# li-kunyi/CUT3R-SLAM

Measured on AMD Instinct MI355X. Metric: frames/sec (ViT pointmap + covisibility-graph tracking step) on 640x480, higher is better.
Workload: dtype f16

## Files before the change

### cut3r_slam_amd/csrc/attention.hip

```cpp
#include <atomic>
#include <cmath>
#include <cstdlib>
#include <type_traits>
#include "common.h"
#include "../../include/cut3r_hip.h"

namespace {

typedef __fp16 fp16x4_t __attribute__((ext_vector_type(4)));

DEVINL void halves(float x, float& lo, float& hi) {
    const auto r = __builtin_amdgcn_permlane32_swap(__float_as_uint(x), __float_as_uint(x), false, false);
    lo = __uint_as_float(r[0]);
    hi = __uint_as_float(r[1]);
}

struct AttnArgs {
    const h16* q; const h16* k; const h16* v; h16* o;
    int Nq, Nk;
    long long q_sb, q_sn, k_sb, k_sn, v_sb, v_sn, o_sb, o_sn;
    float scale_log2;
};

template <int D, int NW>
__global__ __launch_bounds__(NW * 64, (D <= 64 && NW == 4) ? 3 : 1) void attn_kernel(const AttnArgs a) {
    constexpr int NTHR = NW * 64;
    constexpr int KT = 64;
    constexpr int DQ = D / 16;
    constexpr int DP = (D + 31) / 32;
    constexpr int KS_LD = D + 8;
    constexpr int VS_BYTES = (64 * DP) % 128 == 0 ? 64 * DP + 64 : 64 * DP;
    constexpr int V_LD = VS_BYTES / 2;
    constexpr int CHUNKS = KT * (D / 8);
    constexpr int NCH = (CHUNKS + NTHR - 1) / NTHR;
    __shared__ __attribute__((aligned(16))) h16 Ks[KT * KS_LD];
    __shared__ __attribute__((aligned(16))) h16 Vs[KT * V_LD];

    const int tid = threadIdx.x, lane = tid & 63, wave = tid >> 6;
    const int r = lane & 31, hh = lane >> 5;
    const int h = blockIdx.y, b = blockIdx.z;
    const int q0 = blockIdx.x * (32 * NW) + wave * 32;
    const h16* qp = a.q + (size_t)b * a.q_sb + (size_t)h * D;
    const h16* kp = a.k + (size_t)b * a.k_sb + (size_t)h * D;
    const h16* vp = a.v + (size_t)b * a.v_sb + (size_t)h * D;

    for (int i = tid; i < KT * V_LD; i += NTHR) Vs[i] = (h16)0;

    half8_t qf[DQ];
    {
        int qr = q0 + r;
        if (qr > a.Nq - 1) qr = a.Nq - 1;
        const h16* qrow = qp + (size_t)qr * a.q_sn;
#pragma unroll
        for (int s = 0; s < DQ; s++) qf[s] = *reinterpret_cast<const half8_t*>(qrow + 16 * s + 8 * hh);
    }

    f32x16 ot[DP];
#pragma unroll
    for (int d = 0; d < DP; d++)
#pragma unroll
        for (int i = 0; i < 16; i++) ot[d][i] = 0.f;
    float m_run = -INFINITY, l_run = 0.f;
    const bool active = q0 < a.Nq;
    const int extra = (a.Nk > KT && (a.Nk % KT) == 1) ? 1 : 0;
    if (extra) {
        float dot = 0.f;
#pragma unroll
        for (int s = 0; s < DQ; s++) {
            const half8_t k0 = *reinterpret_cast<const half8_t*>(kp + 16 * s + 8 * hh);
#pragma unroll
            for (int j = 0; j < 8; j++) dot = fmaf((float)qf[s][j], (float)k0[j], dot);
        }
        { float d0, d1; halves(dot, d0, d1); dot = d0 + d1; }
        m_run = dot * a.scale_log2;
        l_run = hh == 0 ? 1.f : 0.f;
#pragma unroll
        for (int d = 0; d < DP; d++)
#pragma unroll
            for (int g4 = 0; g4 < 4; g4++) {
                const int dd = d * 32 + 8 * g4 + 4 * hh;
                if (dd < D) {
                    const half4_t v0 = *reinterpret_cast<const half4_t*>(vp + dd);
#pragma unroll
                    for (int e = 0; e < 4; e++) ot[d][4 * g4 + e] = (float)v0[e];
                }
            }
    }

    half8_t rk[NCH], rv[NCH];
    const h16* kptr[NCH];
    const h16* vptr[NCH];
    int kkey[NCH];
#pragma unroll
    for (int c = 0; c < NCH; c++) {
        const int id = tid + c * NTHR;
        const int key = id / (D / 8), ch = id - key * (D / 8);
        kkey[c] = key;
        kptr[c] = kp + (size_t)(extra + key) * a.k_sn + ch * 8;
        vptr[c] = vp + (size_t)(extra + key) * a.v_sn + ch * 8;
    }
    auto load_kv = [&](int t) {
        const int kbase = extra + t * KT;
        const bool full = kbase + KT <= a.Nk;
#pragma unroll
        for (int c = 0; c < NCH; c++) {
// ... 35 lines not shown
        half8_t kf[2][DQ];
#pragma unroll
        for (int kt2 = 0; kt2 < 2; kt2++)
#pragma unroll
            for (int s = 0; s < DQ; s++) kf[kt2][s] = *reinterpret_cast<const half8_t*>(&Ks[(kt2 * 32 + r) * KS_LD + 16 * s + 8 * hh]);
        __builtin_amdgcn_sched_barrier(0);
#pragma unroll
        for (int kt2 = 0; kt2 < 2; kt2++) {
#pragma unroll
            for (int i = 0; i < 16; i++) st[kt2][i] = 0.f;
#pragma unroll
            for (int s = 0; s < DQ; s++) st[kt2] = __builtin_amdgcn_mfma_f32_32x32x16_f16(kf[kt2][s], qf[s], st[kt2], 0, 0, 0);
        }
        const int kbase = extra + t * KT;
        float mloc = -INFINITY;
        if (kbase + KT <= a.Nk) {
#pragma unroll
            for (int kt2 = 0; kt2 < 2; kt2++)
#pragma unroll
                for (int i = 0; i < 16; i++) mloc = fmaxf(mloc, st[kt2][i]);
        } else {
#pragma unroll
            for (int kt2 = 0; kt2 < 2; kt2++)
#pragma unroll
                for (int i = 0; i < 16; i++) {
                    const int key = kbase + kt2 * 32 + (i & 3) + 8 * (i >> 2) + 4 * hh;
                    const float sv = key < a.Nk ? st[kt2][i] : -INFINITY;
                    st[kt2][i] = sv;
                    mloc = fmaxf(mloc, sv);
                }
        }
        { float m0_, m1_; halves(mloc, m0_, m1_); mloc = fmaxf(m0_, m1_) * a.scale_log2; }
        const float m_new = fmaxf(m_run, mloc);
        const bool grew = m_new > m_run;
        const float alpha = __builtin_amdgcn_exp2f(m_run - m_new);
        m_run = m_new;
        float lsum = 0.f;
#pragma unroll
        for (int kt2 = 0; kt2 < 2; kt2++)
#pragma unroll
            for (int i = 0; i < 16; i++) {
                const float p = __builtin_amdgcn_exp2f(fmaf(st[kt2][i], a.scale_log2, -m_new));
                st[kt2][i] = p;
                lsum += p;
            }
        l_run = l_run * alpha + lsum;
        if (__any(grew)) {
#pragma unroll
            for (int d = 0; d < DP; d++)
#pragma unroll
                for (int i = 0; i < 16; i++) ot[d][i] *= alpha;
        }

        const int g16 = lane >> 4, j16 = lane & 15;
#pragma unroll
        for (int kt2 = 0; kt2 < 2; kt2++)
#pragma unroll
            for (int s2 = 0; s2 < 2; s2++) {
                half8_t pf;
#pragma unroll
                for (int j = 0; j < 8; j++) pf[j] = (h16)st[kt2][8 * s2 + j];
#pragma unroll
                for (int d = 0; d < DP; d++) {
                    const int k0 = kt2 * 32 + 16 * s2 + 4 * (g16 >> 1);
                    const int c0 = d * 32 + 16 * (g16 & 1);
                    const h16* vp = &Vs[(k0 + (j16 >> 2)) * V_LD + c0 + 4 * (j16 & 3)];
                    const fp16x4_t lo = __builtin_amdgcn_ds_read_tr16_b64_v4f16((__attribute__((address_space(3))) fp16x4_t*)(vp));
                    const fp16x4_t hi = __builtin_amdgcn_ds_read_tr16_b64_v4f16((__attribute__((address_space(3))) fp16x4_t*)(vp + 8 * V_LD));
                    half8_t vf;
                    __builtin_memcpy(&vf, &lo, 8);
                    __builtin_memcpy(reinterpret_cast<char*>(&vf) + 8, &hi, 8);
                    ot[d] = __builtin_amdgcn_mfma_f32_32x32x16_f16(vf, pf, ot[d], 0, 0, 0);
                }
            }
    }

    float l0_, l1_;
    halves(l_run, l0_, l1_);
    const float l_tot = l0_ + l1_;
    const float inv = 1.0f / l_tot;
    const int qr = q0 + r;
    if (qr < a.Nq) {
        h16* orow = a.o + (size_t)b * a.o_sb + (size_t)qr * a.o_sn + (size_t)h * D;
#pragma unroll
        for (int d = 0; d < DP; d++)
#pragma unroll
            for (int g4 = 0; g4 < 4; g4++) {
                int dd = d * 32 + 8 * g4 + 4 * hh;
                if (dd < D) {
                    half4_t o = {(h16)(ot[d][4 * g4 + 0] * inv), (h16)(ot[d][4 * g4 + 1] * inv), (h16)(ot[d][4 * g4 + 2] * inv),
                                 (h16)(ot[d][4 * g4 + 3] * inv)};
                    *reinterpret_cast<half4_t*>(orow + dd) = o;
                }
            }
    }
}


DEVINL void dma_piece(const char* gbase , unsigned voff, unsigned lds ) {
    asm volatile("s_mov_b32 m0, %2\n\ts_nop 0\n\tglobal_load_lds_dwordx4 %0, %1" ::"v"(voff), "s"(gbase), "s"(lds) : "memory", "m0");
}
DEVINL unsigned lds_addr(const void* p) {
    return (unsigned)(unsigned long long)(__attribute__((address_space(3))) const void*)p;
}

template <int N>
DEVINL void wait_vm() { asm volatile("s_waitcnt vmcnt(%0)" ::"n"(N) : "memory"); }
template <int P, int MAXT>
DEVINL void wait_tiles_ahead(int tiles_ahead) {
    if constexpr (MAXT == 0) wait_vm<0>();
    else {
        if (tiles_ahead >= MAXT) wait_vm<P * MAXT>();
        else wait_tiles_ahead<P, MAXT - 1>(tiles_ahead);
    }
}

template <int D, int QB, int NST, int NW>
__global__ __launch_bounds__(64 * NW, (QB == 1 ? 2 : 1)) void attn_pipe_kernel(const AttnArgs a, const int nblk, const int HB, const int H) {
    constexpr int KT = 64;
    constexpr int PPW = 8 / NW;
    constexpr int AHEAD = NST - 4;
    constexpr int DQ = D / 16;
    constexpr int DP = (D + 31) / 32;
    constexpr int CH = D / 8;
    constexpr int VOFF = KT * 128;
    constexpr int STAGE = 2 * KT * 128;
    static_assert(D % 16 == 0 && D <= 64 && NST >= 4 && (NW == 4 || NW == 8), "head dims 16..64; the ring holds tiles j-1 .. j+2 and NST-4 more in flight");
    __shared__ __attribute__((aligned(1024))) unsigned char smem[NST * STAGE];

    const int tid = threadIdx.x, lane = tid & 63;
    const int wave = __builtin_amdgcn_readfirstlane(tid >> 6);
    const int r = lane & 31, hh = lane >> 5;
    const int L = blockIdx.x;
    const int xb = (L >> 3) % nblk;
    const int bh = ((L >> 3) / nblk) * 8 + (L & 7);
    if (bh >= HB) return;
    const int h = bh % H, b = bh / H;
    const int q0 = xb * (32 * NW * QB) + wave * (32 * QB);
    const h16* qp = a.q + (size_t)b * a.q_sb + (size_t)h * D;
    const h16* kp = a.k + (size_t)b * a.k_sb + (size_t)h * D;
    const h16* vp = a.v + (size_t)b * a.v_sb + (size_t)h * D;
    const bool active = q0 < a.Nq;
    const int extra = (a.Nk > KT && (a.Nk % KT) == 1) ? 1 : 0;
    const int ntiles = (a.Nk - extra + KT - 1) / KT;

    if (CH < 8) {
        for (int i = tid; i < NST * STAGE / 16; i += 64 * NW) *reinterpret_cast<f32x4*>(smem + i * 16) = f32x4{0.f, 0.f, 0.f, 0.f};
        asm volatile("s_waitcnt lgkmcnt(0)" ::: "memory");
        asm volatile("s_barrier" ::: "memory");
    }

    auto lane_src = [&](int c, int row_limit, unsigned& ko, unsigned& vo, bool& kval, bool& vval) {
        const int row = (wave * PPW + c) * 8 + (lane >> 3), slot = lane & 7;
        const int kc = slot ^ ((row >> 1) & 7), vc = slot ^ (((row >> 1) & 1) << 2);
        const int rr = min(row, row_limit);
        ko = (unsigned)rr * (unsigned)(a.k_sn * 2) + kc * 16;
        vo = (unsigned)rr * (unsigned)(a.v_sn * 2) + vc * 16;
        kval = kc < CH;
        vval = vc < CH;
    };
    unsigned koffb[PPW], voffb[PPW];
#pragma unroll
    for (int c = 0; c < PPW; c++) {
        bool kv_, vv_;
        lane_src(c, KT - 1, koffb[c], voffb[c], kv_, vv_);
    }
    const char* ktile = reinterpret_cast<const char*>(kp + (size_t)extra * a.k_sn);
    const char* vtile = reinterpret_cast<const char*>(vp + (size_t)extra * a.v_sn);
    int st_issue = 0;
    auto issue = [&](int t) {
        if (t >= ntiles) return;
        unsigned char* st = smem + st_issue * STAGE;
        st_issue = st_issue + 1 == NST ? 0 : st_issue + 1;
        const int left = a.Nk - (extra + t * KT);
#pragma unroll
        for (int c = 0; c < PPW; c++) {
            unsigned ko = koffb[c], vo = voffb[c];
// ... 190 lines not shown
                    __builtin_amdgcn_sched_group_barrier(0x008, 1, 0);
                    __builtin_amdgcn_sched_group_barrier(0x100, 2, 0);
                    __builtin_amdgcn_sched_group_barrier(0x002, 9, 0);
                }
            }
            int gflag = grew ? 1 : 0;
#pragma unroll
            for (int qb = 0; qb < QB; qb++) {
                typedef unsigned u32x4 __attribute__((ext_vector_type(4)));
                u32x4 p0, p1, p2, p3;
                __builtin_memcpy(&p0, &P[PAR][qb][0][0], 16);
                __builtin_memcpy(&p1, &P[PAR][qb][0][1], 16);
                __builtin_memcpy(&p2, &P[PAR][qb][1][0], 16);
                __builtin_memcpy(&p3, &P[PAR][qb][1][1], 16);
                asm volatile("" : "+v"(gflag) : "v"(p0), "v"(p1), "v"(p2), "v"(p3), "v"(l_run[qb]));
            }
            if (__any(gflag)) {
#pragma unroll
                for (int qb = 0; qb < QB; qb++)
#pragma unroll
                    for (int d = 0; d < DP; d++)
#pragma unroll
                        for (int i = 0; i < 16; i++) ot[qb][d][i] *= alpha[qb];
            }
        }
    };
    using T0 = std::integral_constant<int, 0>;
    using T1 = std::integral_constant<int, 1>;
    using Y = std::true_type;
    using N = std::false_type;

#pragma unroll
    for (int t = 0; t < NST - 3; t++) issue(t);
    {
        wait_tiles_ahead<2 * PPW, AHEAD>(ntiles - 1);
        asm volatile("s_barrier" ::: "memory");
        issue(NST - 3);
        {
            half8_t kf[2][DQ];
#pragma unroll
            for (int kt2 = 0; kt2 < 2; kt2++)
#pragma unroll
                for (int s = 0; s < DQ; s++) kf[kt2][s] = *reinterpret_cast<const half8_t*>(smem + kt2 * 32 * 128 + koff[s]);
#pragma unroll
            for (int kt2 = 0; kt2 < 2; kt2++)
#pragma unroll
                for (int qb = 0; qb < QB; qb++) {
#pragma unroll
                    for (int i = 0; i < 16; i++) S[0][qb][kt2][i] = 0.f;
#pragma unroll
                    for (int s = 0; s < DQ; s++) S[0][qb][kt2] = __builtin_amdgcn_mfma_f32_32x32x16_f16(kf[kt2][s], qf[qb][s], S[0][qb][kt2], 0, 0, 0);
                }
        }
    }
    const bool ragged = extra + ntiles * KT > a.Nk;
    if (ntiles > 1) step(T0{}, N{}, Y{}, Y{}, N{}, 0);
    else if (ragged) step(T0{}, N{}, N{}, Y{}, Y{}, 0);
    else step(T0{}, N{}, N{}, Y{}, N{}, 0);
    int j = 1;
    for (; j + 2 < ntiles; j += 2) {
        step(T1{}, Y{}, Y{}, Y{}, N{}, j);
        step(T0{}, Y{}, Y{}, Y{}, N{}, j + 1);
    }
    if (j + 1 < ntiles) { step(T1{}, Y{}, Y{}, Y{}, N{}, j); j++; }
    if (ntiles > 1) {
        if (ragged) {
            if (j & 1) step(T1{}, Y{}, N{}, Y{}, Y{}, j); else step(T0{}, Y{}, N{}, Y{}, Y{}, j);
        } else {
            if (j & 1) step(T1{}, Y{}, N{}, Y{}, N{}, j); else step(T0{}, Y{}, N{}, Y{}, N{}, j);
        }
        j++;
    }
    if (j & 1) step(T1{}, Y{}, N{}, N{}, N{}, j); else step(T0{}, Y{}, N{}, N{}, N{}, j);

#pragma unroll
    for (int qb = 0; qb < QB; qb++) {
        float l0_, l1_;
        halves(l_run[qb], l0_, l1_);
        const float l_tot = l0_ + l1_;
        const float inv = 1.0f / l_tot;
        const int qr = q0 + qb * 32 + r;
        if (qr < a.Nq) {
            h16* orow = a.o + (size_t)b * a.o_sb + (size_t)qr * a.o_sn + (size_t)h * D;
#pragma unroll
            for (int d = 0; d < DP; d++)
#pragma unroll
                for (int g4 = 0; g4 < 4; g4++) {
                    int dd = d * 32 + 8 * g4 + 4 * hh;
                    if (dd < D) {
                        half4_t o = {(h16)(ot[qb][d][4 * g4 + 0] * inv), (h16)(ot[qb][d][4 * g4 + 1] * inv), (h16)(ot[qb][d][4 * g4 + 2] * inv),
                                     (h16)(ot[qb][d][4 * g4 + 3] * inv)};
                        *reinterpret_cast<half4_t*>(orow + dd) = o;
                    }
                }
        }
    }
}

std::atomic<int> g_attn_variant{[] { const char* e = getenv("CUT3R_ATTN_PIPE"); return e ? atoi(e) : 1; }()};

int attn_instance(int B, int H, int Nq, int D) {
    static const long long nw4_min = [] { const char* e = getenv("CUT3R_ATTN_NW4_MIN"); return e ? atoll(e) : 384LL; }();
    if (D != 16 && D != 32 && D != 48 && D != 64 && D != 128) return 0;
    if ((D == 48 || D == 64) && g_attn_variant.load(std::memory_order_relaxed) != 0) return 104;
    const long long blocks128 = (long long)B * H * ((Nq + 127) / 128);
    return (blocks128 >= nw4_min || D >= 128) ? 4 : 2;
}

template <int D>
int launch_attn(const AttnArgs& a, int B, int H, hipStream_t s) {
    const int inst = attn_instance(B, H, a.Nq, D);
    if constexpr (D == 48 || D == 64) {
        if (inst == 104) {
            const int nblk = (a.Nq + 127) / 128, HB = H * B;
            dim3 grid((unsigned)(((HB + 7) / 8) * 8 * nblk));
            hipLaunchKernelGGL((attn_pipe_kernel<D, 1, 4, 4>), grid, dim3(256), 0, s, a, nblk, HB, H);
            return cut3r_check_launch();
        }
    }
    if (inst == 4) {
        dim3 grid((a.Nq + 127) / 128, H, B);
        hipLaunchKernelGGL((attn_kernel<D, 4>), grid, dim3(256), 0, s, a);
    } else if (inst == 2) {
        dim3 grid((a.Nq + 63) / 64, H, B);
        hipLaunchKernelGGL((attn_kernel<D, 2>), grid, dim3(128), 0, s, a);
    } else {
        return CUT3R_ERR_ARG;
    }
    return cut3r_check_launch();
}

}

extern "C" int cut3r_attention_variant(int v) {
    if (v < 0) return g_attn_variant.load(std::memory_order_relaxed);
    return g_attn_variant.exchange(v ? 1 : 0, std::memory_order_relaxed);
}

extern "C" int cut3r_attention_kernel_for(int B, int H, int Nq, int D) {
    if (B <= 0 || H <= 0 || Nq <= 0) return 0;
    return attn_instance(B, H, Nq, D);
}

extern "C" int cut3r_attention_f16(const void* q, const void* k, const void* v, void* out, int B, int H, int Nq, int Nk, int D,
                                   long long q_sb, long long q_sn, long long k_sb, long long k_sn, long long v_sb, long long v_sn,
                                   long long o_sb, long long o_sn, float scale, void* stream) {
    if (!q || !k || !v || !out || B <= 0 || H <= 0 || Nq <= 0 || Nk <= 0) return CUT3R_ERR_ARG;
    if (((uintptr_t)q | (uintptr_t)k | (uintptr_t)v) & 15) return CUT3R_ERR_ARG;
    if ((uintptr_t)out & 7) return CUT3R_ERR_ARG;
    if ((q_sn | k_sn | v_sn | q_sb | k_sb | v_sb) & 7) return CUT3R_ERR_ARG;
    if ((o_sn | o_sb) & 3) return CUT3R_ERR_ARG;
    if (!(scale > 0.f) || !std::isfinite(scale)) return CUT3R_ERR_ARG;
    AttnArgs a;
    a.q = (const h16*)q; a.k = (const h16*)k; a.v = (const h16*)v; a.o = (h16*)out;
    a.Nq = Nq; a.Nk = Nk;
    a.q_sb = q_sb; a.q_sn = q_sn; a.k_sb = k_sb; a.k_sn = k_sn; a.v_sb = v_sb; a.v_sn = v_sn; a.o_sb = o_sb; a.o_sn = o_sn;
    a.scale_log2 = scale * 1.44269504088896340736f;
    hipStream_t s = (hipStream_t)stream;
    switch (D) {
        case 16: return launch_attn<16>(a, B, H, s);
        case 32: return launch_attn<32>(a, B, H, s);
        case 48: return launch_attn<48>(a, B, H, s);
        case 64: return launch_attn<64>(a, B, H, s);
        case 128: return launch_attn<128>(a, B, H, s);
        default: return CUT3R_ERR_ARG;
    }
}
```

### cut3r_slam_amd/csrc/gemm.hip

```cpp
#include <cstdlib>
#include "common.h"
#include "dpt_tail.h"
#include "../../include/cut3r_hip.h"

namespace {

constexpr int BK = 64;
constexpr int KCH = BK / 8;

struct GemmArgs {
    const h16* A; const h16* B; void* C;
    const float* bias; const void* res1; const void* res2;
    int M, N, K, lda, ldb, ldc, ldr1, ldr2;
    int act, out_f16, res1_f16, res2_f16;
    long long sA, sB, sC, sBias, sR1, sR2;
    int conv_k, H, W, Cin, cstride, Ho, Wo, relu_in;
    int shuf, shuf_cout, shuf_Hin, shuf_Win;
    int swz;
    int prio;
    const long long* rope_pos; const float* rope_table; int rope_cols, rope_pmin, rope_npos, rope_d;
    const float* ln_stats; const float* ln_c; int ln_nslab; float ln_eps;
    float* stats_out; h16* out16; int ld16;
    const float* dpt_w; const float* dpt_b; float* dpt_pts; float* dpt_conf; long long dpt_pts_vs, dpt_conf_vs;
};
// ... 522 lines not shown
    }
#pragma unroll
    for (int p = 0; p < EPI_PASSES; p++) {
        f32x4 r1v[PF];
        auto load_r1 = [&](int i) {
            const int r = r0 + i * RPP;
            const int gm = m0 + p * EPI_ROWS + r;
            return (r < EPI_ROWS && gm < M) ? load_res4(g.res1, g.res1_f16, (size_t)z * g.sR1 + (size_t)gm * g.ldr1 + gn) : zero4;
        };
        if (plain && col_ok && g.res1) {
#pragma unroll
            for (int i = 0; i < PF; i++) r1v[i] = load_r1(i);
        }
        if (p > 0) __syncthreads();
#pragma unroll
        for (int i = 0; i < MT; i++)
#pragma unroll
            for (int j = 0; j < NT; j++)
#pragma unroll
                for (int e = 0; e < 4; e++) {
                    const int r = wm * WM + i * 16 + fq * 4 + e - p * EPI_ROWS;
                    const int c = wn * WN + j * 16 + fr;
                    if (EPI_PASSES == 1 || (r >= 0 && r < EPI_ROWS)) cs[r * CPAD + c] = acc[i][j][e];
                }
        __syncthreads();
        if (col_ok) {
            if (plain) {
#pragma unroll
                for (int i = 0; i < ITER; i++) {
                    const int r = r0 + i * RPP;
                    const int gm = m0 + p * EPI_ROWS + r;
                    f32x4 r1 = zero4;
                    if (g.res1) {
                        r1 = r1v[i % PF];
                        if (i + PF < ITER) r1v[i % PF] = load_r1(i + PF);
                    }
                    if (r < EPI_ROWS && gm < M) {
                        const f32x4 r2 = g.res2 ? load_res4(g.res2, g.res2_f16, (size_t)z * g.sR2 + (size_t)gm * g.ldr2 + gn) : zero4;
                        f32x4 v = *reinterpret_cast<const f32x4*>(cs + r * CPAD + c4);
                        if (g.ln_stats) v = ln_pre4(v, lnp[2 * (p * EPI_ROWS + r)], lnp[2 * (p * EPI_ROWS + r) + 1], *reinterpret_cast<const f32x4*>(g.ln_c + gn));
                        store_out4(g, z, (size_t)gm * g.ldc + gn, fused_finish4(g, v, b4, bias != nullptr, r1, r2));
                    }
                }
            } else {
                for (int r = r0; r < EPI_ROWS; r += RPP) {
                    const int gm = m0 + p * EPI_ROWS + r;
                    if (gm >= M) break;
                    f32x4 v = *reinterpret_cast<const f32x4*>(cs + r * CPAD + c4);
                    const float rs = g.ln_stats ? lnp[2 * (p * EPI_ROWS + r)] : 1.f, rm = g.ln_stats ? lnp[2 * (p * EPI_ROWS + r) + 1] : 0.f;
                    if (gn < g.rope_cols) rope_store4(g, z, bias, gm, gn, cs + r * CPAD, c4, rs, rm);
                    else {
                        if (g.ln_stats) v = ln_pre4(v, rs, rm, *reinterpret_cast<const f32x4*>(g.ln_c + gn));
                        fused_store4(g, z, bias, gm, gn, v);
                    }
                }
            }
        }
    }
}

#define CUT3R_TILE_BOUNDS __launch_bounds__(64 * WAVES_M * WAVES_N, (WAVES_M * WAVES_N == 8 && (BM + BN) * BK * 2 * NSTAGE <= 81920) ? 4 : 1)
template <int BM, int BN, int NSTAGE, int WAVES_M = 2, int WAVES_N = 2, int ADDR = 0, int EPI = 0>
__global__ CUT3R_TILE_BOUNDS void gemm_kernel(const GemmArgs g) {
    gemm_tile_body<BM, BN, NSTAGE, WAVES_M, WAVES_N, ADDR, EPI>(g, blockIdx.x, blockIdx.y, blockIdx.z);
}

static int tile_addr_mode(const GemmArgs& g) {
    static const bool off = [] { const char* e = getenv("CUT3R_GEMM_FASTADDR"); return e && atoi(e) == 0; }();
    if (off || (g.K % BK) != 0) return 0;
    if (g.conv_k == 3) return (g.Cin >= 64 && (g.Cin & (g.Cin - 1)) == 0 && g.K == 9 * g.Cin) ? 2 : 0;
    return 1;
}

struct GemmPairArgs { GemmArgs p[2]; int nblk0; };
template <int BM, int BN, int NSTAGE, int WAVES_M = 2, int WAVES_N = 2, int ADDR = 0, int EPI = 0>
__global__ CUT3R_TILE_BOUNDS void gemm_pair_kernel(const GemmPairArgs a) {
    const int sel = (int)blockIdx.x >= a.nblk0 ? 1 : 0;
    gemm_tile_body<BM, BN, NSTAGE, WAVES_M, WAVES_N, ADDR, EPI>(a.p[sel], blockIdx.x - sel * a.nblk0, 0, 0);
}

#ifndef EPI_UNROLL
#define EPI_UNROLL 1
#endif
template <bool CONV3, bool RELU_IN, bool FAST_DMA = false, int EPI = 0, bool LN = false>
DEVINL void gemm256_body(const GemmArgs& g, const int bx, const int bz) {
    constexpr int UNIT = 128 * BK * 2;
    constexpr int BUF = 4 * UNIT;
    static_assert(!LN || EPI == 1 || EPI == 2 || EPI == 6, "the LayerNorm fold feeds the fp16-output epilogues");
    __shared__ __attribute__((aligned(16))) unsigned char smem[2 * BUF + (LN ? 2 * 1024 : 0)];

    const int tid = threadIdx.x, lane = tid & 63, wave = tid >> 6;
    const int wr = wave >> 2, wc = wave & 3;
    const int z = bz;
    const h16* __restrict__ A = g.A + (size_t)z * g.sA;
    const h16* __restrict__ Bm = g.B + (size_t)z * g.sB;
    const int M = g.M, N = g.N, K = g.K;
    int pid_m, pid_n;
    xcd_tile(bx, (M + 255) / 256, (N + 255) / 256, pid_m, pid_n);
    const int m0 = pid_m * 256, n0 = pid_n * 256;
    const h16* zero = reinterpret_cast<const h16*>(g_zero16);

    const int lrow = lane >> 3;
    const int csrc = (lane & 7) ^ lrow;
    const h16* a_ptr[2][2];
    int a_oy[2][2], a_ox[2][2];
    bool a_ok[2][2];
    const h16* b_ptr[2][2];
    bool b_ok[2][2];
#pragma unroll
    for (int q = 0; q < 2; q++)
#pragma unroll
        for (int i = 0; i < 2; i++) {
            const int u = (wave + 8 * i) * 8 + lrow;
            const int gm = m0 + (u >> 6) * 128 + q * 64 + (u & 63);
            a_ok[q][i] = gm < M;
            if (CONV3) {
                const int gmc = a_ok[q][i] ? gm : 0;
                const int hw = g.Ho * g.Wo;
                const int b = gmc / hw, rem = gmc - b * hw;
                const int oy = rem / g.Wo, ox = rem - oy * g.Wo;
                a_oy[q][i] = oy * g.cstride - 1;
                a_ox[q][i] = ox * g.cstride - 1;
                a_ptr[q][i] = A + (size_t)b * g.H * g.W * g.Cin;
            } else {
                a_oy[q][i] = a_ox[q][i] = 0;
                a_ptr[q][i] = A + (size_t)(a_ok[q][i] ? gm : 0) * g.lda;
            }
            const int gn = n0 + (u >> 5) * 64 + q * 32 + (u & 31);
            b_ok[q][i] = gn < N;
            b_ptr[q][i] = Bm + (size_t)(b_ok[q][i] ? gn : 0) * g.ldb;
        }

    const int nt = (K + BK - 1) / BK;
    constexpr bool fast_dma = FAST_DMA;
    unsigned a_off[2][2], b_off[2][2];
    const h16* a_pc[2][2];
    unsigned a_msk[2][2];
    const int cin_shift = 31 - __builtin_clz((unsigned)(g.Cin > 0 ? g.Cin : 1));
    if (FAST_DMA && CONV3) {
#pragma unroll
        for (int q = 0; q < 2; q++)
#pragma unroll
            for (int i = 0; i < 2; i++) {
                a_pc[q][i] = a_ptr[q][i] + ((ptrdiff_t)a_oy[q][i] * g.W + a_ox[q][i]) * g.Cin + csrc * 8;
                unsigned mk = 0;
#pragma unroll
                for (int t = 0; t < 9; t++) {
                    const int iy = a_oy[q][i] + t / 3, ix = a_ox[q][i] + t % 3;
                    if (a_ok[q][i] && iy >= 0 && iy < g.H && ix >= 0 && ix < g.W) mk |= 1u << t;
                }
                a_msk[q][i] = mk;
            }
    }
#pragma unroll
    for (int q = 0; q < 2; q++)
#pragma unroll
        for (int i = 0; i < 2; i++) {
            const int u = (wave + 8 * i) * 8 + lrow;
            const int gm = min(m0 + (u >> 6) * 128 + q * 64 + (u & 63), M - 1);
            const int gn = min(n0 + (u >> 5) * 64 + q * 32 + (u & 31), N - 1);
            a_off[q][i] = (unsigned)(((size_t)gm * g.lda + csrc * 8) * 2);
            b_off[q][i] = (unsigned)(((size_t)gn * g.ldb + csrc * 8) * 2);
        }
    auto issue_fast = [&](const h16* mat, const unsigned (&off)[2], int kt, int unit) {
        const char* base = reinterpret_cast<const char*>(mat) + (size_t)kt * (BK * 2);
        unsigned char* slot = smem + (kt & 1) * BUF + unit * UNIT;
        const int wave_s = __builtin_amdgcn_readfirstlane(wave);
#pragma unroll
        for (int i = 0; i < 2; i++)
            __builtin_amdgcn_global_load_lds((const __attribute__((address_space(1))) void*)(base + off[i]),
                                             (__attribute__((address_space(3))) void*)(slot + (wave_s + 8 * i) * 1024), 16, 0, 0);
    };
    auto issue_a = [&](int q, int kt, int unit) {
        if (kt >= nt) return;
        if constexpr (fast_dma && !CONV3) { issue_fast(A, a_off[q], kt, unit); return; }
        if constexpr (fast_dma && CONV3) {
            const int k0 = kt * BK;
            const int tap = k0 >> cin_shift;
            const int dy = (tap >= 3) + (tap >= 6), dx = tap - 3 * dy;
            const int delta = (dy * g.W + dx) * g.Cin + (k0 & (g.Cin - 1));
            unsigned char* slot = smem + (kt & 1) * BUF + unit * UNIT;
            const int wave_s = __builtin_amdgcn_readfirstlane(wave);
#pragma unroll
            for (int i = 0; i < 2; i++) {
                const h16* src = ((a_msk[q][i] >> tap) & 1) ? a_pc[q][i] + delta : zero;
                __builtin_amdgcn_global_load_lds((const __attribute__((address_space(1))) void*)src,
                                                 (__attribute__((address_space(3))) void*)(slot + (wave_s + 8 * i) * 1024), 16, 0, 0);
            }
            return;
        }
        unsigned char* slot = smem + (kt & 1) * BUF + unit * UNIT;
        const int k = kt * BK + csrc * 8;
        const bool kok = k < K;
        int ci = 0, dy = 0, dx = 0;
        if (CONV3) {
            const int tap = k / g.Cin;
            ci = k - tap * g.Cin;
            dy = tap / 3; dx = tap - dy * 3;
        }
#pragma unroll
        for (int i = 0; i < 2; i++) {
            const h16* src = zero;
            if (CONV3) {
                const int iy = a_oy[q][i] + dy, ix = a_ox[q][i] + dx;
                if (kok && a_ok[q][i] && iy >= 0 && iy < g.H && ix >= 0 && ix < g.W)
                    src = a_ptr[q][i] + ((size_t)iy * g.W + ix) * g.Cin + ci;
            } else if (kok && a_ok[q][i]) {
                src = a_ptr[q][i] + k;
            }
            __builtin_amdgcn_global_load_lds((const __attribute__((address_space(1))) void*)src,
                                             (__attribute__((address_space(3))) void*)(slot + (wave + 8 * i) * 1024), 16, 0, 0);
        }
    };
    auto issue_b = [&](int q, int kt, int unit) {
        if (kt >= nt) return;
        if constexpr (fast_dma) { issue_fast(Bm, b_off[q], kt, unit); return; }
        unsigned char* slot = smem + (kt & 1) * BUF + unit * UNIT;
        const int k = kt * BK + csrc * 8;
        const bool kok = k < K;
#pragma unroll
        for (int i = 0; i < 2; i++) {
            const h16* src = (kok && b_ok[q][i]) ? b_ptr[q][i] + k : zero;
            __builtin_amdgcn_global_load_lds((const __attribute__((address_space(1))) void*)src,
                                             (__attribute__((address_space(3))) void*)(slot + (wave + 8 * i) * 1024), 16, 0, 0);
        }
    };

    const int fr = lane & 15, fq = lane >> 4;
    const int offk0 = fr * 128 + (((0 + fq) ^ (fr & 7)) << 4);
    const int offk1 = fr * 128 + (((4 + fq) ^ (fr & 7)) << 4);
    const int a_base = wr * 64 * 128;
    const int b_base = wc * 32 * 128;

    f32x4 acc[8][4];
    half8_t fa[4][2], fb0[2][2], fb1[2][2];

    auto read_a = [&](const unsigned char* unit) {
#pragma unroll
        for (int i = 0; i < 4; i++) {
            fa[i][0] = *reinterpret_cast<const half8_t*>(unit + a_base + i * 2048 + offk0);
            fa[i][1] = *reinterpret_cast<const half8_t*>(unit + a_base + i * 2048 + offk1);
            if (RELU_IN) { fa[i][0] = relu8(fa[i][0]); fa[i][1] = relu8(fa[i][1]); }
        }
    };
    auto read_b = [&](const unsigned char* unit, half8_t (&fb)[2][2]) {
#pragma unroll
        for (int j = 0; j < 2; j++) {
            fb[j][0] = *reinterpret_cast<const half8_t*>(unit + b_base + j * 2048 + offk0);
            fb[j][1] = *reinterpret_cast<const half8_t*>(unit + b_base + j * 2048 + offk1);
        }
    };
#define CUT3R_BARRIER() asm volatile("s_barrier" ::: "memory")
#define CUT3R_QUADRANT(I0, J0, FB)                                                                              \
    do {                                                                                                         \
        __builtin_amdgcn_s_setprio(1);                                                                           \
        _Pragma("unroll") for (int kk = 0; kk < 2; kk++)                                                         \
            _Pragma("unroll") for (int i = 0; i < 4; i++)                                                        \
                _Pragma("unroll") for (int j = 0; j < 2; j++)                                                    \
                    acc[I0 + i][J0 + j] = __builtin_amdgcn_mfma_f32_16x16x32_f16(fa[i][kk], FB[j][kk], acc[I0 + i][J0 + j], 0, 0, 0); \
        __builtin_amdgcn_s_setprio(0);                                                                           \
    } while (0)

#ifndef CUT3R_G256_PHASES
#define CUT3R_G256_PHASES 2
#endif
    static_assert(!LN || CUT3R_G256_PHASES == 2, "the LayerNorm fold is wired into the two-phase schedule");
#if CUT3R_G256_PHASES == 2
    LnRow ln_raw;
    if constexpr (LN) {
        if (tid < 256) ln_row_load(g.ln_stats, min(m0 + tid, M - 1), M, g.ln_nslab, ln_raw);
    }
    issue_a(0, 0, 0); issue_b(0, 0, 1); issue_b(1, 0, 2); issue_a(1, 0, 3);
    issue_a(0, 1, 0); issue_b(0, 1, 1); issue_b(1, 1, 2);
#pragma unroll
    for (int i = 0; i < 8; i++)
#pragma unroll
        for (int j = 0; j < 4; j++) acc[i][j] = f32x4{0.f, 0.f, 0.f, 0.f};
    if constexpr (LN) {
        if (tid < 256) {
            float rs_, rm_;
            ln_row_finish(ln_raw, g.ln_nslab, K, g.ln_eps, rs_, rm_);
            *reinterpret_cast<float2*>(smem + 2 * BUF + tid * 8) = float2{rs_, rm_};
        }
        asm volatile("s_waitcnt lgkmcnt(0)" ::: "memory");
    }
    if (nt > 1) wait_vmcnt<6>(); else wait_vmcnt<0>();
    CUT3R_BARRIER();
    if (wr == 1) CUT3R_BARRIER();

    for (int t = 0; t < nt; t++) {
        const unsigned char* buf = smem + (t & 1) * BUF;
        read_a(buf);
        read_b(buf + UNIT, fb0);
        read_b(buf + 2 * UNIT, fb1);
        issue_a(1, t + 1, 3);
        if (t + 1 < nt) wait_vmcnt<8>(); else wait_vmcnt<0>();
        asm volatile("s_waitcnt lgkmcnt(0)" ::: "memory");
        CUT3R_BARRIER();
        CUT3R_QUADRANT(0, 0, fb0);
        CUT3R_QUADRANT(0, 2, fb1);
        CUT3R_BARRIER();
        read_a(buf + 3 * UNIT);
        issue_a(0, t + 2, 0); issue_b(0, t + 2, 1); issue_b(1, t + 2, 2);
        if (t + 2 < nt) wait_vmcnt<8>(); else if (t + 1 < nt) wait_vmcnt<2>(); else wait_vmcnt<0>();
        asm volatile("s_waitcnt lgkmcnt(0)" ::: "memory");
        CUT3R_BARRIER();
        CUT3R_QUADRANT(4, 0, fb0);
        CUT3R_QUADRANT(4, 2, fb1);
        CUT3R_BARRIER();
    }
#else
    issue_a(0, 0, 0); issue_b(0, 0, 1); issue_b(1, 0, 2); issue_a(1, 0, 3);
    issue_a(0, 1, 0); issue_b(0, 1, 1);
#pragma unroll
    for (int i = 0; i < 8; i++)
#pragma unroll
        for (int j = 0; j < 4; j++) acc[i][j] = f32x4{0.f, 0.f, 0.f, 0.f};
    if (nt > 1) wait_vmcnt<4>(); else wait_vmcnt<0>();
    CUT3R_BARRIER();
    if (wr == 1) CUT3R_BARRIER();

    for (int t = 0; t < nt; t++) {
        const unsigned char* buf = smem + (t & 1) * BUF;
        read_a(buf);
        read_b(buf + UNIT, fb0);
        issue_b(1, t + 1, 2);
        CUT3R_BARRIER();
        CUT3R_QUADRANT(0, 0, fb0);
        CUT3R_BARRIER();
        read_b(buf + 2 * UNIT, fb1);
        issue_a(1, t + 1, 3);
        CUT3R_BARRIER();
        CUT3R_QUADRANT(0, 2, fb1);
        CUT3R_BARRIER();
        read_a(buf + 3 * UNIT);
        issue_a(0, t + 2, 0);
        CUT3R_BARRIER();
        CUT3R_QUADRANT(4, 2, fb1);
        CUT3R_BARRIER();
        issue_b(0, t + 2, 1);
        if (t + 2 < nt) wait_vmcnt<4>(); else wait_vmcnt<0>();
        CUT3R_BARRIER();
        CUT3R_QUADRANT(4, 0, fb0);
        CUT3R_BARRIER();
    }
#endif
    if (wr == 0) CUT3R_BARRIER();
#undef CUT3R_QUADRANT

    constexpr int CP = 68;
    float* cs = reinterpret_cast<float*>(smem + wave * 16384);
    const float* bias = g.bias ? g.bias + (size_t)z * g.sBias : nullptr;
    const bool plain = !g.shuf && g.rope_cols == 0;
    const f32x4 zero4 = {0.f, 0.f, 0.f, 0.f};
    const float* lnp = reinterpret_cast<const float*>(smem + 2 * BUF) + wr * 256;
    if constexpr (EPI == 1 || EPI == 2 || EPI == 4 || EPI == 5 || EPI == 6) {
        const int er = lane >> 3, ec = (lane & 7) * 8;
        const int gn = n0 + wc * 64 + ec;
        const bool col_ok = gn + 8 <= N;
        const int gnc = col_ok ? gn : 0;
        const f32x4 b0 = *reinterpret_cast<const f32x4*>(bias + gnc), b1 = *reinterpret_cast<const f32x4*>(bias + gnc + 4);
        f32x4 lc0 = zero4, lc1 = zero4, lpc0 = zero4, lpc1 = zero4;
        if constexpr (LN) { lc0 = *reinterpret_cast<const f32x4*>(g.ln_c + gnc); lc1 = *reinterpret_cast<const f32x4*>(g.ln_c + gnc + 4); }
        const bool rope_here = EPI == 6 && (n0 + wc * 64) < g.rope_cols && col_ok;
        f32x4 pb0 = zero4, pb1 = zero4;
        if (rope_here) {
            const int pc = gnc + ((ec & 16) ? -16 : 16);
            pb0 = *reinterpret_cast<const f32x4*>(bias + pc);
            pb1 = *reinterpret_cast<const f32x4*>(bias + pc + 4);
            if constexpr (LN) { lpc0 = *reinterpret_cast<const f32x4*>(g.ln_c + pc); lpc1 = *reinterpret_cast<const f32x4*>(g.ln_c + pc + 4); }
        }
        constexpr int ROPE_LDS = 48;
        float* tl = cs + 32 * CP;
        int* psl = reinterpret_cast<int*>(tl + ROPE_LDS * 32);
        if (EPI == 6 && __builtin_amdgcn_readfirstlane((n0 + wc * 64) < g.rope_cols)) {
#pragma unroll
            for (int f0 = 0; f0 < ROPE_LDS * 8; f0 += 64) {
                const int f = f0 + lane, p = f >> 3, part = f & 7;
                f32x4 v = zero4;
                if (p < g.rope_npos) v = *reinterpret_cast<const f32x4*>(g.rope_table + (size_t)(part >> 2) * g.rope_npos * 16 + p * 16 + (part & 3) * 4);
                *reinterpret_cast<f32x4*>(tl + p * 32 + part * 4) = v;
            }
#pragma unroll
            for (int i = 0; i < 2; i++) {
                const int r = lane + 64 * i;
                const int gmr = min(m0 + wr * 128 + r, M - 1);
                const longlong2 pp = *reinterpret_cast<const longlong2*>(g.rope_pos + (size_t)gmr * 2);
                long long py = pp.x - g.rope_pmin, px = pp.y - g.rope_pmin;
                py = py < 0 ? 0 : (py >= g.rope_npos ? g.rope_npos - 1 : py);
                px = px < 0 ? 0 : (px >= g.rope_npos ? g.rope_npos - 1 : px);
                psl[r * 2] = (int)py;
                psl[r * 2 + 1] = (int)px;
            }
            asm volatile("s_waitcnt lgkmcnt(0)" ::: "memory");
        }
        h16* crow = (h16*)g.C + (size_t)z * g.sC + (size_t)(m0 + wr * 128 + er) * g.ldc + gnc;
        const size_t step8 = (size_t)8 * g.ldc;
#pragma unroll
        for (int mp = 0; mp < 4; mp++) {
            f32x4 ra[4], rb[4], sa[4], sb[4];
            if (EPI == 5) {
#pragma unroll
                for (int it = 0; it < 4; it++) {
                    const size_t gm = (size_t)min(m0 + wr * 128 + mp * 32 + it * 8 + er, M - 1);
                    const half8_t h1 = *reinterpret_cast<const half8_t*>((const h16*)g.res1 + (size_t)z * g.sR1 + gm * g.ldr1 + gnc);
                    ra[it] = f32x4{(float)h1[0], (float)h1[1], (float)h1[2], (float)h1[3]};
                    rb[it] = f32x4{(float)h1[4], (float)h1[5], (float)h1[6], (float)h1[7]};
                    if (g.res2) {
                        const half8_t h2 = *reinterpret_cast<const half8_t*>((const h16*)g.res2 + (size_t)z * g.sR2 + gm * g.ldr2 + gnc);
                        sa[it] = f32x4{(float)h2[0], (float)h2[1], (float)h2[2], (float)h2[3]};
                        sb[it] = f32x4{(float)h2[4], (float)h2[5], (float)h2[6], (float)h2[7]};
                    }
                }
            }
#pragma unroll
            for (int i = 0; i < 2; i++)
#pragma unroll
                for (int j = 0; j < 4; j++)
#pragma unroll
                    for (int e = 0; e < 4; e++) cs[(i * 16 + fq * 4 + e) * CP + j * 16 + fr] = acc[mp * 2 + i][j][e];
            asm volatile("s_waitcnt lgkmcnt(0)" ::: "memory");
#pragma unroll
            for (int it = 0; it < 4; it++) {
                const int rr = it * 8 + er;
                f32x4 v0 = *reinterpret_cast<const f32x4*>(cs + rr * CP + ec);
                f32x4 v1 = *reinterpret_cast<const f32x4*>(cs + rr * CP + ec + 4);
                float rs = 1.f, rm = 0.f;
                if constexpr (LN) {
                    const float2 pr = *reinterpret_cast<const float2*>(lnp + 2 * (mp * 32 + rr));
                    rs = pr.x; rm = pr.y;
                    v0 = ln_pre4(v0, rs, rm, lc0);
                    v1 = ln_pre4(v1, rs, rm, lc1);
                }
                v0 += b0;
                v1 += b1;
                if (EPI == 2) {
#pragma unroll
                    for (int e = 0; e < 4; e++) { v0[e] = gelu_fast(v0[e]); v1[e] = gelu_fast(v1[e]); }
                }
// ... 648 lines not shown
```

Baseline: 5856.

## Write GEMM256 fp16 epilogues directly from registers and widen attention output stores

Result: no change. 5899, median of 6 (+0.7%).

```diff
diff --git a/cut3r_slam_amd/csrc/attention.hip b/cut3r_slam_amd/csrc/attention.hip
--- a/cut3r_slam_amd/csrc/attention.hip
+++ b/cut3r_slam_amd/csrc/attention.hip
@@ -15,12 +15,49 @@
     hi = __uint_as_float(r[1]);
 }
 
+template <int D, int DP>
+DEVINL void attn_store_row(h16* orow, const f32x16 (&ot)[DP], const float inv, const int hh, const bool wide) {
+    typedef unsigned u32x4 __attribute__((ext_vector_type(4)));
+    typedef unsigned u32x2 __attribute__((ext_vector_type(2)));
+    if (wide) {
+#pragma unroll
+        for (int d = 0; d < DP; d++)
+#pragma unroll
+            for (int g4 = 0; g4 < 4; g4 += 2) {
+                if (d * 32 + 8 * g4 < D) {
+                    const half4_t oa = {(h16)(ot[d][4 * g4 + 0] * inv), (h16)(ot[d][4 * g4 + 1] * inv), (h16)(ot[d][4 * g4 + 2] * inv),
+                                        (h16)(ot[d][4 * g4 + 3] * inv)};
+                    const half4_t ob = {(h16)(ot[d][4 * g4 + 4] * inv), (h16)(ot[d][4 * g4 + 5] * inv), (h16)(ot[d][4 * g4 + 6] * inv),
+                                        (h16)(ot[d][4 * g4 + 7] * inv)};
+                    const u32x2 ua = __builtin_bit_cast(u32x2, oa), ub = __builtin_bit_cast(u32x2, ob);
+                    const auto x = __builtin_amdgcn_permlane32_swap(ua[0], ub[0], false, false);
+                    const auto y = __builtin_amdgcn_permlane32_swap(ua[1], ub[1], false, false);
+                    *reinterpret_cast<u32x4*>(orow + d * 32 + 8 * g4 + 8 * hh) = u32x4{x[0], y[0], x[1], y[1]};
+                }
+            }
+    } else {
+#pragma unroll
+        for (int d = 0; d < DP; d++)
+#pragma unroll
+            for (int g4 = 0; g4 < 4; g4++) {
+                const int dd = d * 32 + 8 * g4 + 4 * hh;
+                if (dd < D) {
+                    const half4_t o = {(h16)(ot[d][4 * g4 + 0] * inv), (h16)(ot[d][4 * g4 + 1] * inv), (h16)(ot[d][4 * g4 + 2] * inv),
+                                       (h16)(ot[d][4 * g4 + 3] * inv)};
+                    *reinterpret_cast<half4_t*>(orow + dd) = o;
+                }
+            }
+    }
+}
+
 struct AttnArgs {
     const h16* q; const h16* k; const h16* v; h16* o;
     int Nq, Nk;
     long long q_sb, q_sn, k_sb, k_sn, v_sb, v_sn, o_sb, o_sn;
     float scale_log2;
 };
+
+DEVINL bool attn_wide_out(const AttnArgs& a) { return (((uintptr_t)a.o >> 1 | a.o_sb | a.o_sn) & 7) == 0; }
 
 template <int D, int NW>
 __global__ __launch_bounds__(NW * 64, (D <= 64 && NW == 4) ? 3 : 1) void attn_kernel(const AttnArgs a) {
@@ -222,17 +259,7 @@
     const int qr = q0 + r;
     if (qr < a.Nq) {
         h16* orow = a.o + (size_t)b * a.o_sb + (size_t)qr * a.o_sn + (size_t)h * D;
-#pragma unroll
-        for (int d = 0; d < DP; d++)
-#pragma unroll
-            for (int g4 = 0; g4 < 4; g4++) {
-                int dd = d * 32 + 8 * g4 + 4 * hh;
-                if (dd < D) {
-                    half4_t o = {(h16)(ot[d][4 * g4 + 0] * inv), (h16)(ot[d][4 * g4 + 1] * inv), (h16)(ot[d][4 * g4 + 2] * inv),
-                                 (h16)(ot[d][4 * g4 + 3] * inv)};
-                    *reinterpret_cast<half4_t*>(orow + dd) = o;
-                }
-            }
+        attn_store_row<D, DP>(orow, ot, inv, hh, attn_wide_out(a));
     }
 }
 
@@ -589,17 +616,7 @@
         const int qr = q0 + qb * 32 + r;
         if (qr < a.Nq) {
             h16* orow = a.o + (size_t)b * a.o_sb + (size_t)qr * a.o_sn + (size_t)h * D;
-#pragma unroll
-            for (int d = 0; d < DP; d++)
-#pragma unroll
-                for (int g4 = 0; g4 < 4; g4++) {
-                    int dd = d * 32 + 8 * g4 + 4 * hh;
-                    if (dd < D) {
-                        half4_t o = {(h16)(ot[qb][d][4 * g4 + 0] * inv), (h16)(ot[qb][d][4 * g4 + 1] * inv), (h16)(ot[qb][d][4 * g4 + 2] * inv),
-                                     (h16)(ot[qb][d][4 * g4 + 3] * inv)};
-                        *reinterpret_cast<half4_t*>(orow + dd) = o;
-                    }
-                }
+            attn_store_row<D, DP>(orow, ot[qb], inv, hh, attn_wide_out(a));
         }
     }
 }
diff --git a/cut3r_slam_amd/csrc/gemm.hip b/cut3r_slam_amd/csrc/gemm.hip
--- a/cut3r_slam_amd/csrc/gemm.hip
+++ b/cut3r_slam_amd/csrc/gemm.hip
@@ -628,10 +628,14 @@
 #ifndef EPI_UNROLL
 #define EPI_UNROLL 1
 #endif
+#ifndef CUT3R_G256_DIRECT
+#define CUT3R_G256_DIRECT ((1 << 2) | (1 << 6) | (1 << 9) | (1 << 10) | (1 << 14))
+#endif
 template <bool CONV3, bool RELU_IN, bool FAST_DMA = false, int EPI = 0, bool LN = false>
 DEVINL void gemm256_body(const GemmArgs& g, const int bx, const int bz) {
     constexpr int UNIT = 128 * BK * 2;
     constexpr int BUF = 4 * UNIT;
+    constexpr bool DIRECT = ((CUT3R_G256_DIRECT >> (EPI + (LN ? 8 : 0))) & 1) && !CONV3 && !RELU_IN && FAST_DMA && (EPI == 1 || EPI == 2 || EPI == 6);
     static_assert(!LN || EPI == 1 || EPI == 2 || EPI == 6, "the LayerNorm fold feeds the fp16-output epilogues");
     __shared__ __attribute__((aligned(16))) unsigned char smem[2 * BUF + (LN ? 2 * 1024 : 0)];
 
@@ -645,6 +649,17 @@
     xcd_tile(bx, (M + 255) / 256, (N + 255) / 256, pid_m, pid_n);
     const int m0 = pid_m * 256, n0 = pid_n * 256;
     const h16* zero = reinterpret_cast<const h16*>(g_zero16);
+
+    auto w_col = [&](int q, int u) -> int {
+        const int v = u & 31;
+        if constexpr (DIRECT) {
+            const int j = v >> 4, f = (v >> 2) & 3, e = v & 3;
+            if constexpr (EPI == 6) return (u >> 5) * 64 + 32 * (f >> 1) + 8 * (f & 1) + 16 * q + 4 * j + e;
+            else return (u >> 5) * 64 + 32 * q + 8 * f + 4 * j + e;
+        } else {
+            return (u >> 5) * 64 + q * 32 + v;
+        }
+    };
 
     const int lrow = lane >> 3;
     const int csrc = (lane & 7) ^ lrow;
@@ -672,7 +687,7 @@
                 a_oy[q][i] = a_ox[q][i] = 0;
                 a_ptr[q][i] = A + (size_t)(a_ok[q][i] ? gm : 0) * g.lda;
             }
-            const int gn = n0 + (u >> 5) * 64 + q * 32 + (u & 31);
+            const int gn = n0 + w_col(q, u);
             b_ok[q][i] = gn < N;
             b_ptr[q][i] = Bm + (size_t)(b_ok[q][i] ? gn : 0) * g.ldb;
         }
@@ -704,7 +719,7 @@
         for (int i = 0; i < 2; i++) {
             const int u = (wave + 8 * i) * 8 + lrow;
             const int gm = min(m0 + (u >> 6) * 128 + q * 64 + (u & 63), M - 1);
-            const int gn = min(n0 + (u >> 5) * 64 + q * 32 + (u & 31), N - 1);
+            const int gn = min(n0 + w_col(q, u), N - 1);
             a_off[q][i] = (unsigned)(((size_t)gm * g.lda + csrc * 8) * 2);
             b_off[q][i] = (unsigned)(((size_t)gn * g.ldb + csrc * 8) * 2);
         }
@@ -803,7 +818,8 @@
         _Pragma("unroll") for (int kk = 0; kk < 2; kk++)                                                         \
             _Pragma("unroll") for (int i = 0; i < 4; i++)                                                        \
                 _Pragma("unroll") for (int j = 0; j < 2; j++)                                                    \
-                    acc[I0 + i][J0 + j] = __builtin_amdgcn_mfma_f32_16x16x32_f16(fa[i][kk], FB[j][kk], acc[I0 + i][J0 + j], 0, 0, 0); \
+                    acc[I0 + i][J0 + j] = DIRECT ? __builtin_amdgcn_mfma_f32_16x16x32_f16(FB[j][kk], fa[i][kk], acc[I0 + i][J0 + j], 0, 0, 0) \
+                                                 : __builtin_amdgcn_mfma_f32_16x16x32_f16(fa[i][kk], FB[j][kk], acc[I0 + i][J0 + j], 0, 0, 0); \
         __builtin_amdgcn_s_setprio(0);                                                                           \
     } while (0)
 
@@ -900,7 +916,104 @@
     const bool plain = !g.shuf && g.rope_cols == 0;
     const f32x4 zero4 = {0.f, 0.f, 0.f, 0.f};
     const float* lnp = reinterpret_cast<const float*>(smem + 2 * BUF) + wr * 256;
-    if constexpr (EPI == 1 || EPI == 2 || EPI == 4 || EPI == 5 || EPI == 6) {
+    if constexpr (DIRECT) {
+        constexpr int CSTEP = EPI == 6 ? 16 : 32;
+        const int gn0 = n0 + wc * 64 + (EPI == 6 ? 32 * (fq >> 1) + 8 * (fq & 1) : 8 * fq);
+        bool col_ok[2];
+        f32x4 bb[2][2], lc[2][2];
+#pragma unroll
+        for (int h = 0; h < 2; h++) {
+            col_ok[h] = gn0 + CSTEP * h + 8 <= N;
+            const int gnc = col_ok[h] ? gn0 + CSTEP * h : 0;
+#pragma unroll
+            for (int k = 0; k < 2; k++) {
+                bb[h][k] = *reinterpret_cast<const f32x4*>(bias + gnc + 4 * k);
+                lc[h][k] = zero4;
+                if constexpr (LN) lc[h][k] = *reinterpret_cast<const f32x4*>(g.ln_c + gnc + 4 * k);
+            }
+        }
+        constexpr int ROPE_LDS = 48;
+        float* tl = cs + 32 * CP;
+        int* psl = reinterpret_cast<int*>(tl + ROPE_LDS * 32);
+        const bool rope_here = EPI == 6 && __builtin_amdgcn_readfirstlane((n0 + wc * 64) < g.rope_cols && n0 + wc * 64 + 64 <= N);
+        if (rope_here) {
+#pragma unroll
+            for (int f0 = 0; f0 < ROPE_LDS * 8; f0 += 64) {
+                const int f = f0 + lane, p = f >> 3, part = f & 7;
+                f32x4 v = zero4;
+                if (p < g.rope_npos) v = *reinterpret_cast<const f32x4*>(g.rope_table + (size_t)(part >> 2) * g.rope_npos * 16 + p * 16 + (part & 3) * 4);
+                *reinterpret_cast<f32x4*>(tl + p * 32 + part * 4) = v;
+            }
+#pragma unroll
+            for (int i = 0; i < 2; i++) {
+                const int r = lane + 64 * i;
+                const int gmr = min(m0 + wr * 128 + r, M - 1);
+                const longlong2 pp = *reinterpret_cast<const longlong2*>(g.rope_pos + (size_t)gmr * 2);
+                long long py = pp.x - g.rope_pmin, px = pp.y - g.rope_pmin;
+                py = py < 0 ? 0 : (py >= g.rope_npos ? g.rope_npos - 1 : py);
+                px = px < 0 ? 0 : (px >= g.rope_npos ? g.rope_npos - 1 : px);
+                psl[r * 2] = (int)py;
+                psl[r * 2 + 1] = (int)px;
+            }
+            asm volatile("s_waitcnt lgkmcnt(0)" ::: "memory");
+        }
+        h16* crow = (h16*)g.C + (size_t)z * g.sC + (size_t)(m0 + wr * 128 + fr) * g.ldc + gn0;
+        const size_t step16 = (size_t)16 * g.ldc;
+#pragma unroll
+        for (int I = 0; I < 8; I++) {
+            const int rl = 16 * I + fr;
+            f32x4 v[2][2];
+            float rs = 1.f, rm = 0.f;
+            if constexpr (LN) {
+                const float2 pr = *reinterpret_cast<const float2*>(lnp + 2 * rl);
+                rs = pr.x; rm = pr.y;
+            }
+#pragma unroll
+            for (int h = 0; h < 2; h++)
+#pragma unroll
+                for (int k = 0; k < 2; k++) {
+                    v[h][k] = acc[I][2 * h + k];
+                    if constexpr (LN) v[h][k] = ln_pre4(v[h][k], rs, rm, lc[h][k]);
+                    v[h][k] += bb[h][k];
+                    if (EPI == 2) {
+#pragma unroll
+                        for (int e = 0; e < 4; e++) v[h][k][e] = gelu_fast(v[h][k][e]);
+                    }
+                }
+            if (EPI == 6 && rope_here) {
+                const int pv = psl[rl * 2 + (fq >> 1)];
+                f32x4 co[2], si[2];
+                if (__builtin_amdgcn_ballot_w64(pv >= ROPE_LDS) == 0) {
+                    const float* ct = tl + pv * 32 + 8 * (fq & 1);
+                    co[0] = *reinterpret_cast<const f32x4*>(ct); co[1] = *reinterpret_cast<const f32x4*>(ct + 4);
+                    si[0] = *reinterpret_cast<const f32x4*>(ct + 16); si[1] = *reinterpret_cast<const f32x4*>(ct + 20);
+                } else {
+                    const float* ct = g.rope_table + (size_t)pv * 16 + 8 * (fq & 1);
+                    const float* st = ct + (size_t)g.rope_npos * 16;
+                    co[0] = *reinterpret_cast<const f32x4*>(ct); co[1] = *reinterpret_cast<const f32x4*>(ct + 4);
+                    si[0] = *reinterpret_cast<const f32x4*>(st); si[1] = *reinterpret_cast<const f32x4*>(st + 4);
+                }
+#pragma unroll
+                for (int k = 0; k < 2; k++)
+#pragma unroll
+                    for (int e = 0; e < 4; e++) {
+                        const float lo = (float)(h16)v[0][k][e], hi = (float)(h16)v[1][k][e];
+                        float t0 = hi * si[k][e], t1 = lo * si[k][e];
+                        asm volatile("" : "+v"(t0), "+v"(t1));
+                        v[0][k][e] = rope_rot(lo, co[k][e], -t0);
+                        v[1][k][e] = rope_rot(hi, co[k][e], t1);
+                    }
+            }
+            if (m0 + wr * 128 + rl < M) {
+#pragma unroll
+                for (int h = 0; h < 2; h++) {
+                    const half8_t o = {(h16)v[h][0][0], (h16)v[h][0][1], (h16)v[h][0][2], (h16)v[h][0][3],
+                                       (h16)v[h][1][0], (h16)v[h][1][1], (h16)v[h][1][2], (h16)v[h][1][3]};
+                    if (col_ok[h]) *reinterpret_cast<half8_t*>(crow + (size_t)I * step16 + CSTEP * h) = o;
+                }
+            }
+        }
+    } else if constexpr (EPI == 1 || EPI == 2 || EPI == 4 || EPI == 5 || EPI == 6) {
         const int er = lane >> 3, ec = (lane & 7) * 8;
         const int gn = n0 + wc * 64 + ec;
         const bool col_ok = gn + 8 <= N;
```
